# ai4r/Gesture-Generation-from-Trimodal-Context

Measured on AMD Instinct MI355X. Metric: training clips/sec (34-frame, 27-dim pose), post-warm-up GAN iteration, higher is better.
Workload: dtype f32; 1 GPU; multimodal_context GAN training iteration (BASELINE.json configs[1]), epoch > loss_warmup; batch_per_gpu=128, global_batch=128, frames=34, pose_dim=27, audio_samples=36267, n_words=20000, hipgraph=True, parallelism=dp1

## Files before the change

gesture-generation-from-trimodal-context_amd/_lib.py:

```python
import ctypes as C
import os

_HERE = os.path.dirname(os.path.abspath(__file__))
LIB_PATH = os.environ.get("TG_LIB_PATH") or os.path.join(_HERE, "libtrimodal_hip.so")


class Window(C.Structure):
    _fields_ = [("ptr", C.c_void_p), ("batch_stride", C.c_int64), ("row_stride", C.c_int64), ("rows_in", C.c_int32),
                ("rows_out", C.c_int32), ("row_step", C.c_int32), ("shift", C.c_int32), ("dil", C.c_int32),
                ("cw", C.c_int32), ("K", C.c_int32)]


P, I32, I64, F32, U32 = C.c_void_p, C.c_int32, C.c_int64, C.c_float, C.c_uint32
WP = C.POINTER(Window)


class NtProblem(C.Structure):
    _fields_ = [("A", Window), ("Bw", P), ("ldb", I64), ("b_seg_k", I32), ("reserved", I32), ("b_seg_stride", I64), ("bias", P), ("C", P),
                ("c_batch_stride", I64), ("c_row_stride", I64), ("c_rows_out", I32), ("M", I32), ("N", I32), ("act_slope", F32),
                ("accumulate", I32), ("out_scale", P), ("b_planes", P), ("b_plane_stride", I64), ("b_rows", I32), ("b_row0", I32),
                ("gate", P), ("res", P), ("C2", P), ("res_slope", F32), ("drop_site", U32), ("drop_state", P), ("drop_index0", I64),
                ("drop_p", F32), ("reserved4", I32), ("b_planes_kind", I32), ("reserved5", I32), ("b_inv_scale", P), ("a_row_scale", P), ("a_rowmax", P), ("c_rowmax", P), ("c2_rowmax", P), ("a_rowmax_rows", I32), ("reserved6", I32)]


# ... 24 lines not shown
    "tg_gemm_tn": [P, I64, WP, P, I64, I32, I32, I32, P, P, I64, P],
    "tg_colsum": [P, I64, I32, I32, P, I32, P],
    "tg_gru_forward": [P, I64, P, P, P, P, P, P, I64, I32, I32, I32, P],
    "tg_gru_backward": [P, P, P, I64, P, P, P, P, I64, P, I32, I32, I32, P],
    "tg_gru_h64_forward": [P, I64, P, P, P, P, P, P, I64, P, P, I32, I32, P],
    "tg_gru_h64_backward": [P, P, P, P, I64, P, P, P, P, I64, I32, I32, P],
    "tg_gru_forward_cluster": [P, I64, P, P, P, P, P, P, I64, P, P, P, I64, I32, I32, I32, P],
    "tg_gru_forward_cluster_rows": [P, I64, P, P, P, P, P, P, I64, P, P, P, I64, I32, I32, I32, I32, I32, P],
    "tg_gru_forward_vec": [P, I64, P, P, P, P, P, P, I64, I32, I32, I32, P],
    "tg_gru_backward_cluster": [P, P, P, P, I64, P, P, P, P, I64, P, I64, I32, I32, I32, P],
    "tg_gru_backward_cluster_stats": [P, P, P, P, I64, P, P, P, P, I64, P, I64, I32, I32, I32, P, I64, P, P, P],
    "tg_bn_train_stats": [P, I32, I32, I32, P, P, P, P, P, P, F32, F32, I32, P],
    "tg_bn_eval_stats": [P, P, I32, F32, P, P, P],
    "tg_bn_train_fused": [P, P, I32, I32, I32, P, P, P, P, P, P, P, F32, F32, F32, I32, P],
    "tg_bn_apply": [P, P, I32, I32, I32, P, P, P, P, F32, P],
    "tg_bn2_train": [P, P, I32, I32, I32, P, I64, P, P, P, P, P, P, P, F32, F32, F32, I32, P],
    "tg_bn2_backward": [P, P, P, I32, I32, I32, P, P, P, P, F32, P, I64, P, P, P],
    "tg_bn_backward": [P, P, P, I32, I32, P, P, P, P, F32, P, P, P, P],
    "tg_wav_front_stats": [P, I64, I32, I32, P, P, I32, I32, I32, P, I64, P, P, P, P, P, P, F32, F32, I32, P],
    "tg_wav_front_apply": [P, I64, I32, I32, P, P, I32, I32, I32, P, P, P, P, F32, P, P, P],
    "tg_wav_front_backward": [P, P, P, I64, I32, I32, P, P, I32, I32, I32, P, P, P, P, F32, P, I64, P, P, P, P, P],
    "tg_wav_front_backward_fused": [P, I32, P, P, P, I64, I32, I32, P, P, I32, I32, I32, P, P, P, P, F32, P, I64, P, P, P, P, P],
    "tg_speaker_fwd": [P, P, I32, P, P, P, P, P, P, P, P, P, P, P, P, I32, P, I64, I32, P, U32, P],
    "tg_speaker_bwd": [P, P, P, P, P, P, P, P, I32, P, P, P, P, P, P, P, P, P, P, I32, P],
    "tg_wav_conv2_wgrad": [P, P, I32, I32, I32, P, I64, P, P, P],
    "tg_out_mlp_compose": [P, P, P, P, I32, I32, I32, I32, P, P, P, P],
    "tg_out_mlp_param_grads": [P, P, P, P, P, I32, I32, I32, I32, P, P, P, P, P],
    "tg_zero": [P, I64, P],
    "tg_permute3_batch": [P, I32, I32, P],
    "tg_add_relu": [P, P, P, I64, P],
    "tg_act_mask_bwd": [P, P, P, F32, P, I64, P],
    "tg_act_mask_bwd2": [P, P, P, P, F32, P, P, I64, P],
    "tg_embed_gather_drop": [P, P, P, I32, I32, I32, F32, P, U32, P],
    "tg_d_preconv_bwd": [P] * 26 + [I32, P, I64, I32, I32, P],
    "tg_d_preconv_fwd": [P] * 27 + [I64, I32, I32, F32, F32, P],
    "tg_iter_head": [P, P, P, P, P, P, I64, I32, I32, I32, I32, I32, P, P, P, P, I32, P, U32, P, P, P],
    "tg_act_mask_bwd_drop": [P, P, F32, P, U32, I64, F32, P, I64, P],
    "tg_act_mask_bwd2_drop": [P, P, P, F32, P, U32, I64, F32, P, P, I64, P],
    "tg_mul": [P, P, P, I64, P],
    "tg_axpy": [P, P, F32, I32, I64, P],
    "tg_copy2d": [P, I64, P, I64, I32, I32, I32, P],
    "tg_repeat_rows": [P, I64, P, I64, I32, I32, I32, P],
    "tg_sum_rows": [P, I64, P, I64, I32, I32, I32, I32, P],
    "tg_add_halves": [P, P, I32, I32, P],
    "tg_sum_parts": [P, I64, I32, P, I64, P],
    "tg_narrow8_pair": [P, P, P, P, P, I32, I32, P],
    "tg_dup_halves": [P, P, I32, I32, P],
    "tg_make_pre_seq": [P, P, I32, I32, I32, I32, P],
    "tg_embed_gather": [P, P, P, I32, I32, I32, P],
    "tg_assemble_batch": [P, P, P, P, P, P, P, P, P, P, I32, I32, I32, I32, I32, I32, P, P, P, P, P],
    "tg_embed_scatter_add": [P, P, P, I32, I32, I32, P],
    "tg_permute3": [P, P, I32, I32, I32, I32, I32, I32, P],
    "tg_conv_dgrad_pack": [P, P, I32, I32, I32, I32, P],
    "tg_weight_norm_fwd": [P, P, P, I32, I32, I32, P],
    "tg_weight_norm_fwd_batch": [I32, C.POINTER(P), C.POINTER(P), C.POINTER(P), C.POINTER(P), I32, I32, I32, P],
    "tg_weight_norm_bwd": [P, P, P, P, P, I32, I32, I32, P],
    "tg_weight_norm_bwd_batch": [I32, C.POINTER(P), C.POINTER(P), C.POINTER(P), C.POINTER(P), C.POINTER(P), I32, I32, I32, P],
    "tg_rng_advance": [P, P],
    "tg_iter_begin": [P, P, P, P, P],
    "tg_dropout_mask": [P, I64, F32, P, U32, P],
    "tg_dropout_apply": [P, P, P, I64, F32, P, U32, P],
    "tg_normal": [P, I64, P, U32, P],
    "tg_randperm": [P, I32, P, U32, P],
    "tg_gather_i64": [P, P, P, I32, P],
    "tg_reparam_fwd": [P, P, P, P, I64, P],
    "tg_reparam_bwd": [P, P, P, P, P, I64, P],
# ... 138 lines not shown
```

gesture-generation-from-trimodal-context_amd/engine.py:

```python

import os
import zlib

import torch

from . import layers as L
from . import ops, _lib
from .ops import Win
from .params import ParamSlab

WAV_CONVS = ((0, 16, 1, 5, 1600), (3, 32, 16, 6, 0), (6, 64, 32, 6, 0), (9, 32, 64, 6, 0))
WAV_KW = 15


class DeviceRNG:

    def __init__(self, seed, device):
        self.state = ops.new_rng_state(seed, device)
        self._sites = {}

    def site(self, name):
        sid = self._sites.get(name)
        if sid is None:
            sid = (zlib.crc32(name.encode()) & 0x7FFFFFFF) or 1
# ... 81 lines not shown
        self.p_drop = module.dropout_prob
        self.pose_dim = module.pose_dim
        self.T = module.pre_length + module.gen_length
        ctx = module.input_context
        assert ctx in ("both", "audio", "text", "none"), ctx
        self.use_audio, self.use_text = ctx in ("both", "audio"), ctx in ("both", "text")
        self.z_mode = None if not module.z_obj else ("speaker" if module.speaker_embedding is not None else "random")
        D = self.pose_dim
        self.c_audio = D + 1
        self.c_text = self.c_audio + 32 * self.use_audio
        self.c_z = self.c_text + 32 * self.use_text
        self.in_size = self.c_z + (16 if self.z_mode else 0)

    def forward(self, pre_seq, in_text, in_audio, vid, *, training, groups=1, save=False, inject=None, tag="g", save_rows=None, out_into=None,
                side_work=None, side_head=None):
        P, G, Bf = self.views()
        Bs, T = in_text.shape
        H, D = self.H, self.pose_dim
        assert T == self.T and pre_seq.shape == (Bs, T, D + 1) and Bs % groups == 0
        tp = {"Bs": Bs, "groups": groups, "training": training}
        in_size = self.in_size
        pre_in_place = (pre_seq.stride() == (T * in_size, in_size, 1) and pre_seq.storage_offset() == 0 and
                        pre_seq.untyped_storage().nbytes() >= Bs * T * in_size * 4)
        in_data = pre_seq.as_strided((Bs, T, in_size), (T * in_size, in_size, 1)) if pre_in_place else L.empty(Bs, T, in_size, like=pre_seq)
        fork = L.Fork(pre_seq.device, enabled=(self.use_side_stream and self.use_audio) or self._audio_fork_on())
        self._side_work_ran = False
        self._w21_early = None
        L.prep_zone("pre_join")
        if self.use_audio:
            self._audio_fwd(P, Bf, in_audio, in_data, self.c_audio, tp, fork, training, groups, side_work, side_head)
        elif training and self.use_text:
            self._audio_fwd(P, Bf, in_audio, L.empty(Bs, T, 32, like=pre_seq), 0, {}, fork, training, groups, side_work, side_head)
        if self.use_text:
            self._text_fwd(P, in_text, in_data, tp, training, inject, tag)
        mu = logvar = z = None
        z_in_place = False
        if self.z_mode == "speaker":
            assert vid is not None
            draw = None
            if inject is not None and f"{tag}.eps" in inject:
                eps = inject[f"{tag}.eps"].contiguous()
            elif ops.SPEAKER_FUSED:
                eps, draw = L.empty(Bs, 16, like=pre_seq), (self.rng.state, self.rng.site(f"{tag}.eps"))
            else:
                eps = ops.normal(L.empty(Bs, 16, like=pre_seq), self.rng.state, self.rng.site(f"{tag}.eps"))
            if ops.SPEAKER_FUSED:
                se, zc, mu, logvar, z = ops.speaker_fwd(P["speaker_embedding.0.weight"], vid.contiguous(), P["speaker_embedding.1.weight"],
                                                        P["speaker_embedding.1.bias"], P["speaker_mu.weight"], P["speaker_mu.bias"],
                                                        P["speaker_logvar.weight"], P["speaker_logvar.bias"], eps,
                                                        rep=in_data.view(Bs * T, in_size)[:, self.c_z:], T=T, draw=draw)
                z_in_place = True
            else:
                se = ops.embed_gather(P["speaker_embedding.0.weight"], vid.contiguous(), L.empty(Bs, 16, like=pre_seq))
                zc = L.linear_fwd(se, P["speaker_embedding.1.weight"], P["speaker_embedding.1.bias"])
                mu = L.linear_fwd(zc, P["speaker_mu.weight"], P["speaker_mu.bias"])
                logvar = L.linear_fwd(zc, P["speaker_logvar.weight"], P["speaker_logvar.bias"])
                z = ops.reparam_fwd(mu, logvar, eps, torch.empty_like(mu))
            tp.update(se=se, zc=zc, mu=mu, logvar=logvar, eps=eps, vid=vid)
        elif self.z_mode == "random":
            if inject is not None and f"{tag}.z" in inject:
                z = inject[f"{tag}.z"].contiguous()
            else:
                z = ops.normal(L.empty(Bs, 16, like=pre_seq), self.rng.state, self.rng.site(f"{tag}.z"))

        fork.join()
        L.prep_zone("post_join")
        flat_in = in_data.view(Bs * T, in_size)
# ... 44 lines not shown
            wp = L.pack_conv_weight(P[f"{fe}.{idx}.weight"])
            last = idx == 9
            if last and shared:
                Lo = L.conv_out_len(x.shape[1], WAV_KW, stride, pad)
                assert Lo == T, f"audio length gives {Lo} frames, expected {T}"
                a_win = Win.conv(x, WAV_KW, stride=stride, pad=pad, rows_out=Lo)
                probs = []
                for g in range(groups):
                    o = in_data[g * Ba:(g + 1) * Ba, :, ca:ca + 32]
                    probs.append(dict(A=a_win, W=wp, bias=P[f"{fe}.{idx}.bias"], out=o, c_batch_stride=o.stride(0), c_row_stride=o.stride(1), c_rows_out=Lo))
                ops.gemm_nt_group(probs)
                wav.append((x, None, None))
                break
            out = in_data[:, :, ca:ca + 32] if last else None
            c = L.conv_fwd(x, wp, P[f"{fe}.{idx}.bias"], WAV_KW, stride=stride, pad=pad, out=out)
            if last:
                assert c.shape[1] == T, f"audio length gives {c.shape[1]} frames, expected {T}"
                wav.append((x, None, None))
                break
            y, st = L.bn_fwd(c, P[f"{fe}.{idx + 1}.weight"], P[f"{fe}.{idx + 1}.bias"], Bf[f"{fe}.{idx + 1}.running_mean"],
                             Bf[f"{fe}.{idx + 1}.running_var"], Bf[f"{fe}.{idx + 1}.num_batches_tracked"],
                             training=training, groups=1 if shared else groups, act_slope=0.3,
                             repeats=groups if shared else 1)
            wav.append((x, st, c.shape[1]))
            x = y
        if side_work is not None and fork.enabled:
            side_work()
            self._side_work_ran = True
        if fork.enabled and ops.OUT_MLP_COMPOSED and self.early_out_compose:
            self._w21_early = L.frozen(("w21", P["out.0.weight"].data_ptr()), lambda: ops.out_mlp_compose(P["out.0.weight"], P["out.0.bias"], P["out.2.weight"], P["out.2.bias"], dup=2))
        fork.__exit__(None, None, None)
        tp["wav"], tp["wav_shared"] = wav, shared

    def _text_fwd(self, P, in_text, in_data, tp, training, inject, tag):
        Bs, T, in_size = in_data.shape
        te = "text_encoder"
        E = P[f"{te}.embedding.weight"].shape[1]
        if (training and self.tcn_drop_regen and Bs * T >= 8192 and E % 4 == 0 and P[f"{te}.embedding.weight"].data_ptr() % 16 == 0 and
                not (inject is not None and f"{tag}.emb_drop" in inject)):
            cur, emb_mask = ops.embed_gather_drop(P[f"{te}.embedding.weight"], in_text.contiguous().view(-1), L.empty(Bs, T, E, like=in_data), 0.1,
                                                  self.rng.state, self.rng.site(f"{tag}.emb_drop"))
        else:
            emb = ops.embed_gather(P[f"{te}.embedding.weight"], in_text.contiguous().view(-1), L.empty(Bs, T, E, like=in_data))
            cur, emb_mask = self._drop(f"{tag}.emb_drop", emb, 0.1, inject) if training else (emb, None)
        names = [f"{te}.tcn.network.{i}.{c}" for i in range(self.n_layers) for c in ("conv1", "conv2")]
        wps, wts = L.frozen(("tcn_wn", P[names[0] + ".weight_v"].data_ptr(), training),
                            lambda: ops.weight_norm_fwd_batch([P[n + ".weight_v"] for n in names], [P[n + ".weight_g"] for n in names], want_t=training))
        Co_w = wps.shape[1]
        w_pl = ops.split_planes(wps.view(len(names) * Co_w, wps.shape[2])) if (ops.GEMM_PLANES and Bs * T >= 8192) else None
        sites = [f"{tag}.tcn{i}.drop{ci + 1}" for i in range(self.n_layers) for ci in range(2)]
        masks = [None] * len(sites)
        if training:
            if inject is not None and all(sn in inject for sn in sites):
                masks = [inject[sn].contiguous() for sn in sites]
            elif self.p_drop > 0.0 and self.tcn_drop_regen and Bs * T >= 8192 and wps.shape[1] % 4 == 0:
                per = Bs * T * wps.shape[1]
                site = self.rng.site(f"{tag}.tcn.drop")
                masks = [inject[sn].contiguous() if (inject is not None and sn in inject) else
                         ops.Drop(self.rng.state, site, self.p_drop, (Bs, T, wps.shape[1]), index0=j * per) for j, sn in enumerate(sites)]
            elif self.p_drop > 0.0:
                drawn = ops.dropout_mask(L.empty(len(sites), Bs, T, wps.shape[1], like=in_data), self.p_drop, self.rng.state,
                                         self.rng.site(f"{tag}.tcn.drop"))
                masks = [inject[sn].contiguous() if (inject is not None and sn in inject) else drawn[j] for j, sn in enumerate(sites)]
        tcn = []
        fuse_res = wps.shape[1] == cur.shape[2] and cur.is_contiguous() and ops.nt_ext_supported(
            Win.conv(cur, 2, pad=1, dil=1, rows_out=T), wps[0], cur, c_batch_stride=cur.stride(0), c_row_stride=cur.stride(1), c_rows_out=T)
        chain = (w_pl is not None and w_pl.kind == "h2" and fuse_res and cur.is_contiguous()
                 and ops.nt_kernel_plan([dict(A=Win.conv(cur, 2, pad=1, dil=1, rows_out=T), W=wps[0], bias=None, out=cur, c_batch_stride=cur.stride(0),
                                              c_row_stride=cur.stride(1), c_rows_out=T, w_planes=w_pl, a_rowmax=cur.view(-1))])[0] == 2)
        if chain:
            rmax = ops.zeros(1 + 2 * self.n_layers, Bs * T, device=cur.device)
            rm_in = ops.win_row_absmax(Win.conv(cur, 2, pad=1, dil=1, rows_out=T), out=rmax[0])
        for i in range(self.n_layers):
            d = 2 ** i
            blk = {"x": cur, "d": d}
            h = cur
            y = None
            for ci in range(2):
                j = 2 * i + ci
                m = masks[j]
                if m is not None:
                    assert m.shape == (Bs, T, wps.shape[1]), (sites[j], m.shape)
                sc = {}
                if chain:
                    rm_o1 = rmax[1 + self.n_layers + i]
                    sc = dict(a_rowmax=rm_in, out_rowmax=rm_o1) if ci == 0 else dict(a_rowmax=rm_o1, out2_rowmax=rmax[1 + i])
                if ci == 1 and fuse_res:
                    y = torch.empty_like(cur)
                    o = L.conv_fwd(h, wps[j], P[names[j] + ".bias"], 2, pad=d, dil=d, rows_out=T, act_slope=0.0, out_scale=m, res=cur, out2=y,
                                   res_slope=0.0, w_planes=w_pl, w_row0=j * Co_w, **sc)
                    if chain:
                        rm_in = rmax[1 + i]
                else:
                    o = L.conv_fwd(h, wps[j], P[names[j] + ".bias"], 2, pad=d, dil=d, rows_out=T, act_slope=0.0, out_scale=m, w_planes=w_pl,
                                   w_row0=j * Co_w, **sc)
                blk[f"in{ci}"], blk[f"wt{ci}"], blk[f"o{ci}"], blk[f"m{ci}"] = h, (wts[j] if wts is not None else None), o, m
# ... 403 lines not shown
```

gesture-generation-from-trimodal-context_amd/ops.py:

```python
import ctypes as C

import contextlib
import os

import torch

from . import _lib
from ._lib import Window, call


def _stream():
    return C.c_void_p(torch.cuda.current_stream().cuda_stream)


def _f32(t, name="tensor"):
    if not (isinstance(t, torch.Tensor) and t.is_cuda and t.dtype == torch.float32):
        raise TypeError(f"{name}: expected a CUDA float32 tensor, got {type(t).__name__} "
                        f"{getattr(t, 'dtype', None)} {getattr(t, 'device', None)}")
    return t


def _p(t):
    return C.c_void_p(t.data_ptr()) if t is not None else C.c_void_p(0)

# ... 1210 lines not shown

def embed_gather(table, idx, out):
    _flat(table, "table"); _i64(idx, "idx"); _flat(out, "out")
    n_rows, D = table.shape
    assert out.numel() == idx.numel() * D
    call("tg_embed_gather", _p(table), _p(idx), _p(out), idx.numel(), D, n_rows, _stream()); return out


def assemble_batch(rec, out_text, out_audio, out_vec, out_vid, *, remove_word_timing=False):
    B, n_poses = out_text.shape
    A = out_audio.shape[1]
    Dp = out_vec.shape[2]
    assert out_text.dtype == torch.int64 and out_vid.dtype == torch.int64 and out_text.is_contiguous() and out_audio.is_contiguous() and out_vec.is_contiguous()
    assert tuple(out_audio.shape) == (B, A) and tuple(out_vec.shape) == (B, n_poses, Dp) and out_vid.numel() == B
    _f32(out_audio, "out_audio"); _f32(out_vec, "out_vec"); _f32(rec["audio"], "audio"); _f32(rec["vec"], "vec")
    Wmax = rec["word_idx"].shape[1]
    assert rec["audio_off"].numel() == B + 1 and rec["vec_off"].numel() == B + 1 and tuple(rec["word_idx"].shape) == (B, Wmax) == tuple(rec["word_onset"].shape)
    assert rec["word_idx"].dtype == torch.int64 and rec["word_onset"].dtype == torch.float64 and rec["times"].dtype == torch.float64
    assert rec["n_words"].dtype == torch.int32 and rec["n_ext"].dtype == torch.int32 and rec["vid"].dtype == torch.int64
    assert rec["audio"].numel() >= 1 and rec["vec"].numel() >= B * n_poses * Dp
    call("tg_assemble_batch", _p(rec["audio"]), _p(rec["audio_off"]), _p(rec["vec"]), _p(rec["vec_off"]), _p(rec["word_idx"]), _p(rec["word_onset"]),
         _p(rec["n_words"]), _p(rec["times"]), _p(rec["n_ext"]), _p(rec["vid"]), B, Wmax, n_poses, Dp, A, int(bool(remove_word_timing)),
         _p(out_text), _p(out_audio), _p(out_vec), _p(out_vid), _stream())


def embed_gather_drop(table, idx, out, p, state, site):
    _flat(table, "table"); _i64(idx, "idx"); _flat(out, "out")
    n_rows, D = table.shape
    assert out.numel() == idx.numel() * D and D % 4 == 0
    call("tg_embed_gather_drop", _p(table), _p(idx), _p(out), idx.numel(), D, n_rows, float(p), _p(_i64(state, "rng_state")), int(site), _stream())
    return out, Drop(state, site, p, out.shape)


def embed_scatter_add(dout, idx, dtable):
    _flat(dout, "dout"); _i64(idx, "idx"); _flat(dtable, "dtable")
    n_rows, D = dtable.shape
    assert dout.numel() == idx.numel() * D
    call("tg_embed_scatter_add", _p(dout), _p(idx), _p(dtable), idx.numel(), D, n_rows, _stream()); return dtable


def permute3(x, out, perm):
    _flat(x, "in"); _flat(out, "out"); assert x.dim() == 3 and out.numel() == x.numel()
    call("tg_permute3", _p(x), _p(out), *x.shape, *perm, _stream()); return out


def permute3_batch(desc, n_jobs, total_workgroups):
    assert desc.dtype == torch.int64 and desc.is_cuda and desc.is_contiguous() and tuple(desc.shape) == (n_jobs, 10)
    call("tg_permute3_batch", C.c_void_p(desc.data_ptr()), int(n_jobs), int(total_workgroups), _stream())


def conv_dgrad_pack(w, out, stride):
    _flat(w, "w"); _flat(out, "out"); Co, Ci, kw = w.shape
    J = (kw + stride - 1) // stride
    assert out.numel() == stride * Ci * J * Co
    call("tg_conv_dgrad_pack", _p(w), _p(out), Co, Ci, kw, stride, _stream()); return out


def weight_norm_fwd(v, g, w_packed):
    _flat(v, "v"); _flat(g, "g"); _flat(w_packed, "w"); Co, Ci, kw = v.shape
    assert g.numel() == Co and w_packed.numel() == v.numel()
    call("tg_weight_norm_fwd", _p(v), _p(g), _p(w_packed), Co, Ci, kw, _stream()); return w_packed


def weight_norm_fwd_batch(vs, gs, want_t=True):
    n = len(vs)
    Co, Ci, kw = vs[0].shape
# ... 660 lines not shown
```

include/trimodal_hip.h:

```cpp
#ifndef TRIMODAL_HIP_H
#define TRIMODAL_HIP_H

#include <stdint.h>

#ifdef __cplusplus
extern "C" {
#endif

#define TG_ABI_VERSION 11

int tg_version(void);

int tg_set_deterministic(int32_t on);
int tg_get_deterministic(void);
int tg_set_tn_workgroup_cap(int32_t n);
int tg_get_tn_workgroup_cap(void);
const char* tg_last_error(void);

int tg_set_math_mode(int32_t mode);
int tg_get_math_mode(void);

typedef struct tg_window {
    const float* ptr;
    int64_t batch_stride;
// ... 198 lines not shown
int tg_wav_conv2_wgrad(const float* dc2, const float* act, int32_t B, int32_t T1, int32_t T2, float* ws, int64_t ws_floats, float* dW2,
                       float* db2, void* stream);

int tg_add_relu(const float* a, const float* b, float* y, int64_t n, void* stream);
int tg_act_mask_bwd2(const float* dy, const float* y, const float* o, const float* mask, float slope, float* dsum, float* dc, int64_t n, void* stream);
int tg_act_mask_bwd(const float* dy, const float* y, const float* mask, float slope, float* dx, int64_t n,
                    void* stream);
int tg_act_mask_bwd_drop(const float* dy, const float* y, float p, const uint64_t* rng_state, uint32_t site, int64_t index0, float slope,
                         float* dx, int64_t n, void* stream);
int tg_act_mask_bwd2_drop(const float* dy, const float* y, const float* o, float p, const uint64_t* rng_state, uint32_t site, int64_t index0,
                          float slope, float* dsum, float* dc, int64_t n, void* stream);
int tg_mul(const float* x, const float* mask, float* y, int64_t n, void* stream);
int tg_zero(void* p, int64_t bytes, void* stream);
int tg_axpy(const float* x, float* y, float alpha, int32_t accumulate, int64_t n, void* stream);
int tg_copy2d(const float* src, int64_t lds, float* dst, int64_t ldd, int32_t rows, int32_t cols,
              int32_t accumulate, void* stream);
int tg_repeat_rows(const float* src, int64_t lds, float* dst, int64_t ldd, int32_t B, int32_t T, int32_t cols,
                   void* stream);
int tg_sum_rows(const float* src, int64_t lds, float* dst, int64_t ldd, int32_t B, int32_t T, int32_t cols,
                int32_t accumulate, void* stream);
int tg_add_halves(const float* y, float* o, int32_t M, int32_t H, void* stream);
int tg_sum_parts(const float* parts, int64_t stride, int32_t n_parts, float* out, int64_t n, void* stream);
int tg_narrow8_pair(const float* a0, const float* a1, const float* w0, const float* w1, float* out, int32_t M, int32_t K, void* stream);
int tg_dup_halves(const float* d_o, float* dy, int32_t M, int32_t H, void* stream);
int tg_make_pre_seq(const float* target, float* pre, int32_t B, int32_t T, int32_t D, int32_t n_pre, void* stream);
int tg_assemble_batch(const float* audio_raw, const int64_t* audio_off, const float* vec_raw, const int64_t* vec_off, const int64_t* word_idx,
                      const double* word_onset, const int32_t* n_words, const double* times, const int32_t* n_ext, const int64_t* vid_in, int32_t B, int32_t Wmax,
                      int32_t n_poses, int32_t pose_floats, int32_t audio_len, int32_t remove_word_timing, int64_t* out_text, float* out_audio,
                      float* out_vec, int64_t* out_vid, void* stream);
int tg_embed_gather(const float* table, const int64_t* idx, float* out, int32_t n_idx, int32_t D, int32_t n_rows,
                    void* stream);
int tg_embed_gather_drop(const float* table, const int64_t* idx, float* out, int32_t n_idx, int32_t D, int32_t n_rows, float p,
                         const uint64_t* rng_state, uint32_t site, void* stream);
int tg_embed_scatter_add(const float* dout, const int64_t* idx, float* dtable, int32_t n_idx, int32_t D,
                         int32_t n_rows, void* stream);
int tg_permute3(const float* in, float* out, int32_t d0, int32_t d1, int32_t d2, int32_t p0, int32_t p1,
                int32_t p2, void* stream);

int tg_permute3_batch(const int64_t* desc, int32_t n_jobs, int32_t total_workgroups, void* stream);
int tg_conv_dgrad_pack(const float* w, float* out, int32_t Co, int32_t Ci, int32_t kw, int32_t s, void* stream);

int tg_weight_norm_fwd(const float* v, const float* g, float* w_packed, int32_t Co, int32_t Ci, int32_t kw,
                       void* stream);
int tg_weight_norm_fwd_batch(int32_t n, const float* const* v, const float* const* g, float* const* w_packed, float* const* w_t,
                             int32_t Co, int32_t Ci, int32_t kw, void* stream);
int tg_weight_norm_bwd(const float* dw_packed, const float* v, const float* g, float* dg, float* dv, int32_t Co,
                       int32_t Ci, int32_t kw, void* stream);
int tg_weight_norm_bwd_batch(int32_t n, const float* const* dw_packed, const float* const* v, const float* const* g, float* const* dg,
                             float* const* dv, int32_t Co, int32_t Ci, int32_t kw, void* stream);

int tg_rng_advance(uint64_t* rng_state, void* stream);
int tg_iter_begin(uint64_t* rng_a, uint64_t* rng_b, int32_t* adam_step_a, int32_t* adam_step_b, void* stream);
int tg_iter_head(uint64_t* rng_a, uint64_t* rng_b, int32_t* adam_step_a, int32_t* adam_step_b, const float* target, float* pre_stacked, int64_t pre_ld,
                 int32_t B, int32_t T, int32_t D, int32_t n_pre, int32_t copies, const int64_t* text, int64_t* text_stacked, const int64_t* vid,
                 int64_t* vid_stacked, int32_t permute_last, const int64_t* perm_in, uint32_t perm_site, int64_t* perm_out, float* target_copy,
                 void* stream);
int tg_dropout_mask(float* mask, int64_t n, float p, const uint64_t* rng_state, uint32_t site, void* stream);
int tg_dropout_apply(const float* x, float* y, float* mask, int64_t n, float p, const uint64_t* rng_state, uint32_t site,
                     void* stream);
int tg_normal(float* out, int64_t n, const uint64_t* rng_state, uint32_t site, void* stream);
int tg_randperm(int64_t* out, int32_t n, const uint64_t* rng_state, uint32_t site, void* stream);
int tg_gather_i64(const int64_t* src, const int64_t* perm, int64_t* out, int32_t n, void* stream);

int tg_reparam_fwd(const float* mu, const float* logvar, const float* eps, float* z, int64_t n, void* stream);
int tg_reparam_bwd(const float* dz, const float* logvar, const float* eps, float* dmu, float* dlogvar, int64_t n,
                   void* stream);
// ... 137 lines not shown
```

Before: 29610 clips/s.

## Fuse text TCN forward blocks and decoder into one persistent LDS-resident kernel

Adds a single HIP kernel that runs all four text-encoder TCN residual blocks (8 dilated conv layers with bias, ReLU, dropout and residual) plus the 32-wide decoder for two clips per workgroup. Activations stay in LDS as split fp16 hi/lo planes and feed MFMA instructions, replacing the per-layer GEMM launches and their global-memory round trips. It writes the tape tensors the backward pass needs. The cost is a large-LDS kernel with one workgroup per CU, only 64 workgroups for batch 128, and a fixed shape envelope that falls back to the old path otherwise.

```diff
diff --git a/gesture-generation-from-trimodal-context_amd/_lib.py b/gesture-generation-from-trimodal-context_amd/_lib.py
--- a/gesture-generation-from-trimodal-context_amd/_lib.py
+++ b/gesture-generation-from-trimodal-context_amd/_lib.py
@@ -80,6 +80,7 @@
     "tg_act_mask_bwd": [P, P, P, F32, P, I64, P],
     "tg_act_mask_bwd2": [P, P, P, P, F32, P, P, I64, P],
     "tg_embed_gather_drop": [P, P, P, I32, I32, I32, F32, P, U32, P],
+    "tg_tcn_fwd_fused": [P, P, I64, I32, P, C.POINTER(P), P, P, P, U32, F32, I32, I32, I32, I32, P, P, P, I32, I32, P, I64, P],
     "tg_d_preconv_bwd": [P] * 26 + [I32, P, I64, I32, I32, P],
     "tg_d_preconv_fwd": [P] * 27 + [I64, I32, I32, F32, F32, P],
     "tg_iter_head": [P, P, P, P, P, P, I64, I32, I32, I32, I32, I32, P, P, P, P, I32, P, U32, P, P, P],
diff --git a/gesture-generation-from-trimodal-context_amd/csrc/tcn_fused.hip b/gesture-generation-from-trimodal-context_amd/csrc/tcn_fused.hip
--- /dev/null
+++ b/gesture-generation-from-trimodal-context_amd/csrc/tcn_fused.hip
@@ -0,0 +1,313 @@
+#include "common.hpp"
+#include <stdlib.h>
+#include <type_traits>
+
+namespace tg {
+
+constexpr int TF_T = 34, TF_C = 300, TF_R = 2, TF_ROWS = TF_R * TF_T, TF_MT = 5, TF_NTILES = 19, TF_BLOCKS = 4, TF_E = 32;
+constexpr int TF_ROWB = TF_C * 2;
+constexpr int TF_PLANE = TF_ROWS * TF_ROWB;
+constexpr int TF_X_OFF = 0, TF_PL_OFF = TF_ROWS * TF_C * 4, TF_ZERO_OFF = TF_PL_OFF + 2 * TF_PLANE, TF_RMAX_OFF = TF_ZERO_OFF + 16;
+constexpr int TF_LDS = TF_RMAX_OFF + 2 * TF_ROWS * 4;
+constexpr int TF_Q_TAP = TF_C / 4;
+static_assert(TF_LDS <= 163840 && TF_PL_OFF % 16 == 0 && TF_PLANE % 8 == 0 && TF_ROWB % 8 == 0, "LDS layout");
+
+typedef unsigned tf_u32x2 __attribute__((ext_vector_type(2)));
+typedef unsigned tf_u32x4 __attribute__((ext_vector_type(4)));
+
+struct TcnArgs {
+    const float* x0;
+    const unsigned char* wpl;
+    long wplane_b;
+    unsigned wslab_b;
+    int wzero_row;
+    const float* winv;
+    const float* bias[2 * TF_BLOCKS];
+    const float* dec_w;
+    const float* dec_b;
+    const uint64_t* drop;
+    unsigned site;
+    float p;
+    int clips;
+    float *o0, *o1, *y;
+    int save0, save1;
+    float* out;
+    long out_ld;
+};
+
+struct TfW { tg_f16x8 hi, lo; };
+
+template <int NJ>
+__device__ __forceinline__ void tcn_fwd_fused_body(const TcnArgs& a, unsigned char* const smem) {
+    float* const xres = reinterpret_cast<float*>(smem + TF_X_OFF);
+    unsigned char* const pl = smem + TF_PL_OFF;
+    unsigned* const rmax = reinterpret_cast<unsigned*>(smem + TF_RMAX_OFF);
+    constexpr int ZREL = TF_ZERO_OFF - TF_PL_OFF;
+    const int t = threadIdx.x, lane = t & 63;
+    const int wave = __builtin_amdgcn_readfirstlane(t >> 6);
+    const int r16 = lane & 15, kq = lane >> 4;
+    const int clip0 = blockIdx.x * TF_R;
+    const int nclip = a.clips - clip0 < TF_R ? a.clips - clip0 : TF_R;
+
+    auto store_planes = [&](int row, int col, const f32x4 v, float s) __attribute__((always_inline)) {
+        unsigned h0, l0, h1, l1;
+        h2_split2(v[0] * s, v[1] * s, h0, l0);
+        h2_split2(v[2] * s, v[3] * s, h1, l1);
+        unsigned char* const q = pl + row * TF_ROWB + col * 2;
+        *reinterpret_cast<tf_u32x2*>(q) = tf_u32x2{h0, h1};
+        *reinterpret_cast<tf_u32x2*>(q + TF_PLANE) = tf_u32x2{l0, l1};
+    };
+    auto absmax4 = [](unsigned m, const f32x4 v) __attribute__((always_inline)) {
+#pragma unroll
+        for (int q = 0; q < 4; ++q) { const float f = v[q]; const unsigned b = __float_as_uint(f) & 0x7fffffffu; m = m > b ? m : b; }
+        return m;
+    };
+
+    {
+        const f32x4* __restrict__ src = reinterpret_cast<const f32x4*>(a.x0 + (long)clip0 * (TF_T * TF_C));
+        const int live = nclip * (TF_T * TF_C / 4);
+        for (int i = t; i < TF_ROWS * TF_C / 4; i += 512) reinterpret_cast<f32x4*>(xres)[i] = i < live ? src[i] : f32x4{0.f, 0.f, 0.f, 0.f};
+        if (t < 4) reinterpret_cast<unsigned*>(smem + TF_ZERO_OFF)[t] = 0u;
+        if (t < TF_ROWS) rmax[t] = 0u;
+    }
+    __syncthreads();
+    for (int row = wave; row < TF_ROWS; row += 8) {
+        const float* xr = xres + row * TF_C;
+        const bool two = lane + 64 < TF_C / 4;
+        const f32x4 v0 = *reinterpret_cast<const f32x4*>(xr + 4 * lane);
+        const f32x4 v1 = two ? *reinterpret_cast<const f32x4*>(xr + 4 * (lane + 64)) : f32x4{0.f, 0.f, 0.f, 0.f};
+        const unsigned mx = wave_max_u32(absmax4(absmax4(0u, v0), v1));
+        const float s = h2_scale_of_exp(h2_exp_of_bits(mx));
+        if (lane == 0) rmax[TF_ROWS + row] = mx;
+        store_planes(row, 4 * lane, v0, s);
+        if (two) store_planes(row, 4 * (lane + 64), v1, s);
+    }
+    __syncthreads();
+
+    int rowoff1[TF_MT];
+    int tl[TF_MT];
+    int goff[TF_MT];
+    bool rowok[TF_MT], saved[TF_MT], gok[TF_MT];
+#pragma unroll
+    for (int i = 0; i < TF_MT; ++i) {
+        const int m = 16 * i + r16;
+        rowok[i] = m < TF_ROWS;
+        const int mm = rowok[i] ? m : 0;
+        const int c = mm >= TF_T ? 1 : 0;
+        tl[i] = mm - c * TF_T;
+        rowoff1[i] = rowok[i] ? m * TF_ROWB : -1;
+        gok[i] = rowok[i] && c < nclip;
+        const int clip = gok[i] ? clip0 + c : 0;
+        saved[i] = gok[i] && clip >= a.save0 && clip < a.save1;
+        goff[i] = (clip * TF_T + tl[i]) * TF_C;
+    }
+    const long per = (long)a.clips * (TF_T * TF_C);
+    const bool drop_on = a.drop != nullptr && a.p > 0.f;
+
+    f32x4 acc[2][TF_MT][NJ];
+
+    for (int j = 0; j < 2 * TF_BLOCKS; ++j) {
+        const int d = 1 << (j >> 1);
+        const bool second = j & 1;
+        int rowoff0[TF_MT];
+#pragma unroll
+        for (int i = 0; i < TF_MT; ++i) rowoff0[i] = (rowok[i] && tl[i] >= d) ? rowoff1[i] - d * TF_ROWB : -1;
+        unsigned woff[NJ];
+#pragma unroll
+        for (int jn = 0; jn < NJ; ++jn) {
+            const int n = 16 * (wave + 8 * jn) + r16;
+            woff[jn] = (unsigned)(n < TF_C ? j * TF_C + n : a.wzero_row) * 64u + (unsigned)kq * 16u;
+        }
+        auto load_w = [&](int s, TfW (&w)[NJ]) __attribute__((always_inline)) {
+            const unsigned char* __restrict__ base = a.wpl + (size_t)s * a.wslab_b;
+#pragma unroll
+            for (int jn = 0; jn < NJ; ++jn) {
+                w[jn].hi = *reinterpret_cast<const tg_f16x8*>(base + woff[jn]);
+                w[jn].lo = *reinterpret_cast<const tg_f16x8*>(base + a.wplane_b + woff[jn]);
+            }
+        };
+        auto slab = [&](auto tap_c, int s, const TfW (&w)[NJ]) __attribute__((always_inline)) {
+            constexpr int TAP = decltype(tap_c)::value;
+            int cb[2];
+            bool ok[2];
+#pragma unroll
+            for (int h = 0; h < 2; ++h) {
+                const int q = 8 * s + 2 * kq + h;
+                ok[h] = TAP == 0 ? q < TF_Q_TAP : (q >= TF_Q_TAP && q < 2 * TF_Q_TAP);
+                cb[h] = (q - TAP * TF_Q_TAP) * 8;
+            }
+#pragma unroll
+            for (int i = 0; i < TF_MT; ++i) {
+                const int ro = TAP ? rowoff1[i] : rowoff0[i];
+                tf_u32x2 xh[2], xl[2];
+#pragma unroll
+                for (int h = 0; h < 2; ++h) {
+                    const bool v = ok[h] && ro >= 0;
+                    xh[h] = *reinterpret_cast<const tf_u32x2*>(pl + (v ? ro + cb[h] : ZREL));
+                    xl[h] = *reinterpret_cast<const tf_u32x2*>(pl + (v ? ro + cb[h] + TF_PLANE : ZREL));
+                }
+                const tg_f16x8 fh = __builtin_bit_cast(tg_f16x8, tf_u32x4{xh[0][0], xh[0][1], xh[1][0], xh[1][1]});
+                const tg_f16x8 fl = __builtin_bit_cast(tg_f16x8, tf_u32x4{xl[0][0], xl[0][1], xl[1][0], xl[1][1]});
+#pragma unroll
+                for (int jn = 0; jn < NJ; ++jn) acc[TAP][i][jn] = __builtin_amdgcn_mfma_f32_16x16x32_f16(w[jn].lo, fh, acc[TAP][i][jn], 0, 0, 0);
+#pragma unroll
+                for (int jn = 0; jn < NJ; ++jn) acc[TAP][i][jn] = __builtin_amdgcn_mfma_f32_16x16x32_f16(w[jn].hi, fl, acc[TAP][i][jn], 0, 0, 0);
+#pragma unroll
+                for (int jn = 0; jn < NJ; ++jn) acc[TAP][i][jn] = __builtin_amdgcn_mfma_f32_16x16x32_f16(w[jn].hi, fh, acc[TAP][i][jn], 0, 0, 0);
+            }
+        };
+#pragma unroll
+        for (int q = 0; q < 2; ++q)
+#pragma unroll
+            for (int i = 0; i < TF_MT; ++i)
+#pragma unroll
+                for (int jn = 0; jn < NJ; ++jn) acc[q][i][jn] = f32x4{0.f, 0.f, 0.f, 0.f};
+
+        using tap0 = std::integral_constant<int, 0>;
+        using tap1 = std::integral_constant<int, 1>;
+        TfW w0[NJ], w1[NJ];
+        load_w(0, w0);
+        for (int s = 0; s < 10; s += 2) {
+            load_w(s + 1, w1);
+            slab(tap0{}, s, w0);
+            load_w(s + 2 < 10 ? s + 2 : 9, w0);
+            slab(tap0{}, s + 1, w1);
+        }
+        for (int s = 9; s < 19; s += 2) {
+            load_w(s + 1, w1);
+            slab(tap1{}, s, w0);
+            load_w(s + 2 < 19 ? s + 2 : 18, w0);
+            slab(tap1{}, s + 1, w1);
+        }
+
+        const unsigned* const rm_in = rmax + ((j + 1) & 1) * TF_ROWS;
+        unsigned* const rm_out = rmax + (j & 1) * TF_ROWS;
+        const float* __restrict__ bias = a.bias[j];
+        const float* __restrict__ winv = a.winv + j * TF_C;
+        float* __restrict__ const tape0 = (second ? a.o1 : a.o0) + (long)(j >> 1) * per;
+        float* __restrict__ const tape_y = a.y + (long)(j >> 1) * per;
+#pragma unroll
+        for (int i = 0; i < TF_MT; ++i) {
+            const int m = rowok[i] ? 16 * i + r16 : 0;
+            const float inv1 = h2_inv_of_exp(h2_exp_of_bits(rm_in[m]));
+            const float inv0 = h2_inv_of_exp(h2_exp_of_bits(rm_in[tl[i] >= d ? m - d : m]));
+            unsigned mx = 0u;
+#pragma unroll
+            for (int jn = 0; jn < NJ; ++jn) {
+                const int n = 16 * (wave + 8 * jn) + 4 * kq;
+                const bool cok = n < TF_C;
+                const int nn = cok ? n : 0;
+                const f32x4 iw = *reinterpret_cast<const f32x4*>(winv + nn);
+                const f32x4 bv = *reinterpret_cast<const f32x4*>(bias + nn);
+                f32x4 v = (acc[0][i][jn] * inv0) * iw + (acc[1][i][jn] * inv1) * iw + bv;
+#pragma unroll
+                for (int q = 0; q < 4; ++q) v[q] = v[q] > 0.f ? v[q] : 0.f;
+                if (drop_on) v *= dropout_scale4(a.drop, a.site, a.p, (unsigned long)(j * per + goff[i] + nn) >> 2);
+                if (saved[i] && cok) *reinterpret_cast<f32x4*>(tape0 + goff[i] + nn) = v;
+                if (second) {
+                    float* const xp = xres + m * TF_C + nn;
+                    const f32x4 x = *reinterpret_cast<const f32x4*>(xp);
+                    v += x;
+#pragma unroll
+                    for (int q = 0; q < 4; ++q) v[q] = v[q] > 0.f ? v[q] : 0.f;
+                    if (rowok[i] && cok) *reinterpret_cast<f32x4*>(xp) = v;
+                    if (saved[i] && cok) *reinterpret_cast<f32x4*>(tape_y + goff[i] + nn) = v;
+                }
+                if (cok) mx = absmax4(mx, v);
+                acc[1][i][jn] = v;
+            }
+            unsigned o = (unsigned)__shfl_xor((int)mx, 16, 64); mx = mx > o ? mx : o;
+            o = (unsigned)__shfl_xor((int)mx, 32, 64); mx = mx > o ? mx : o;
+            if (kq == 0 && rowok[i]) atomicMax(rm_out + m, mx);
+        }
+        __syncthreads();
+        if (j == 2 * TF_BLOCKS - 1) break;
+        if (t < TF_ROWS) rmax[((j + 1) & 1) * TF_ROWS + t] = 0u;
+#pragma unroll
+        for (int i = 0; i < TF_MT; ++i) {
+            const int m = rowok[i] ? 16 * i + r16 : 0;
+            const float s = h2_scale_of_exp(h2_exp_of_bits(rm_out[m]));
+#pragma unroll
+            for (int jn = 0; jn < NJ; ++jn) {
+                const int n = 16 * (wave + 8 * jn) + 4 * kq;
+                if (rowok[i] && n < TF_C) store_planes(m, n, acc[1][i][jn], s);
+            }
+        }
+        __syncthreads();
+    }
+
+    {
+        const int c = t & 31, mg = t >> 5;
+        const float* __restrict__ wr = a.dec_w + c * TF_C;
+        float s[TF_MT];
+        int mrow[TF_MT];
+#pragma unroll
+        for (int k = 0; k < TF_MT; ++k) { s[k] = 0.f; const int m = mg + 16 * k; mrow[k] = (m < TF_ROWS ? m : 0) * TF_C; }
+        for (int k4 = 0; k4 < TF_C; k4 += 4) {
+            const f32x4 w = *reinterpret_cast<const f32x4*>(wr + k4);
+#pragma unroll
+            for (int k = 0; k < TF_MT; ++k) {
+                const f32x4 x = *reinterpret_cast<const f32x4*>(xres + mrow[k] + k4);
+                s[k] = fmaf(w[0], x[0], s[k]); s[k] = fmaf(w[1], x[1], s[k]); s[k] = fmaf(w[2], x[2], s[k]); s[k] = fmaf(w[3], x[3], s[k]);
+            }
+        }
+        const float b = a.dec_b[c];
+#pragma unroll
+        for (int k = 0; k < TF_MT; ++k) {
+            const int m = mg + 16 * k;
+            const int cl = m >= TF_T ? 1 : 0;
+            if (m < TF_ROWS && cl < nclip) a.out[((long)(clip0 + cl) * TF_T + (m - cl * TF_T)) * a.out_ld + c] = s[k] + b;
+        }
+    }
+}
+
+__global__ __launch_bounds__(512, 1) void tcn_fwd_fused_kernel(const TcnArgs a) {
+    __shared__ __attribute__((aligned(16))) unsigned char smem[TF_LDS];
+    if (__builtin_amdgcn_readfirstlane(threadIdx.x >> 6) + 16 < TF_NTILES) tcn_fwd_fused_body<3>(a, smem);
+    else tcn_fwd_fused_body<2>(a, smem);
+}
+
+}
+
+using namespace tg;
+
+extern "C" int tg_get_math_mode(void);
+
+static bool tcn_fused_envelope(int T, int C, int n_blocks) { return T == TF_T && C == TF_C && n_blocks == TF_BLOCKS && tg_get_math_mode() == 0; }
+
+extern "C" int tg_tcn_fwd_fused(const float* x0, const void* w_planes, int64_t w_plane_stride, int32_t w_rows, const float* w_inv, const float* const* biases,
+                                const float* dec_w, const float* dec_b, const uint64_t* rng_state, uint32_t site, float p, int32_t clips, int32_t T,
+                                int32_t C, int32_t n_blocks, float* o0, float* o1, float* y, int32_t save_row0, int32_t save_rows, float* out,
+                                int64_t out_ld, void* stream) {
+    TG_REQUIRE(x0 && w_planes && w_inv && biases && dec_w && dec_b && out, "tg_tcn_fwd_fused: null argument");
+    TG_REQUIRE(clips > 0 && clips <= (1 << 16), "tg_tcn_fwd_fused: clips must be in [1, 2^16]");
+    TG_REQUIRE(tcn_fused_envelope(T, C, n_blocks), "tg_tcn_fwd_fused: envelope is T = %d, C = %d, %d blocks, fp32-accurate mode", TF_T, TF_C, TF_BLOCKS);
+    constexpr int cwp = (2 * TF_C + 31) / 32 * 32;
+    TG_REQUIRE(w_rows == 2 * TF_BLOCKS * TF_C && w_plane_stride == (int64_t)(w_rows + 1) * cwp,
+               "tg_tcn_fwd_fused: the weight planes must hold %d rows of %d columns (fp16 x 2, slab-tiled)", 2 * TF_BLOCKS * TF_C, 2 * TF_C);
+    TG_REQUIRE(p >= 0.f && p < 1.f && (p == 0.f || rng_state), "tg_tcn_fwd_fused: 0 <= p < 1, and a Philox state when p > 0");
+    TG_REQUIRE(save_row0 >= 0 && save_rows >= 0 && (int64_t)save_row0 + save_rows <= clips, "tg_tcn_fwd_fused: taped clips outside the batch");
+    TG_REQUIRE(save_rows == 0 || (o0 && o1 && y), "tg_tcn_fwd_fused: taped clips need o0 / o1 / y");
+    TG_REQUIRE(out_ld >= TF_E, "tg_tcn_fwd_fused: out_ld below the decoder width");
+    TG_REQUIRE(aligned16(x0) && aligned16(w_planes) && aligned16(w_inv) && aligned16(dec_w) && aligned16(o0) && aligned16(o1) && aligned16(y),
+               "tg_tcn_fwd_fused: 16-byte aligned operands");
+    TcnArgs a;
+    for (int j = 0; j < 2 * TF_BLOCKS; ++j) {
+        TG_REQUIRE(biases[j] && aligned16(biases[j]), "tg_tcn_fwd_fused: bias %d null or misaligned", j);
+        a.bias[j] = biases[j];
+    }
+    a.x0 = x0;
+    a.wpl = static_cast<const unsigned char*>(w_planes);
+    a.wplane_b = (long)w_plane_stride * 2;
+    a.wslab_b = (unsigned)(w_rows + 1) * 64u;
+    a.wzero_row = w_rows;
+    a.winv = w_inv;
+    a.dec_w = dec_w; a.dec_b = dec_b;
+    a.drop = p > 0.f ? rng_state : nullptr;
+    a.site = site; a.p = p; a.clips = clips;
+    a.o0 = o0; a.o1 = o1; a.y = y;
+    a.save0 = save_row0; a.save1 = save_row0 + save_rows;
+    a.out = out; a.out_ld = out_ld;
+    hipLaunchKernelGGL(tcn_fwd_fused_kernel, dim3((clips + TF_R - 1) / TF_R), dim3(512), 0, static_cast<hipStream_t>(stream), a);
+    return check_launch("tg_tcn_fwd_fused");
+}
diff --git a/gesture-generation-from-trimodal-context_amd/engine.py b/gesture-generation-from-trimodal-context_amd/engine.py
--- a/gesture-generation-from-trimodal-context_amd/engine.py
+++ b/gesture-generation-from-trimodal-context_amd/engine.py
@@ -137,7 +137,7 @@
         elif training and self.use_text:
             self._audio_fwd(P, Bf, in_audio, L.empty(Bs, T, 32, like=pre_seq), 0, {}, fork, training, groups, side_work, side_head)
         if self.use_text:
-            self._text_fwd(P, in_text, in_data, tp, training, inject, tag)
+            self._text_fwd(P, in_text, in_data, tp, training, inject, tag, save, save_rows)
         mu = logvar = z = None
         z_in_place = False
         if self.z_mode == "speaker":
@@ -248,7 +248,7 @@
         fork.__exit__(None, None, None)
         tp["wav"], tp["wav_shared"] = wav, shared
 
-    def _text_fwd(self, P, in_text, in_data, tp, training, inject, tag):
+    def _text_fwd(self, P, in_text, in_data, tp, training, inject, tag, save=True, save_rows=None):
         Bs, T, in_size = in_data.shape
         te = "text_encoder"
         E = P[f"{te}.embedding.weight"].shape[1]
@@ -278,6 +278,23 @@
                 drawn = ops.dropout_mask(L.empty(len(sites), Bs, T, wps.shape[1], like=in_data), self.p_drop, self.rng.state,
                                          self.rng.site(f"{tag}.tcn.drop"))
                 masks = [inject[sn].contiguous() if (inject is not None and sn in inject) else drawn[j] for j, sn in enumerate(sites)]
+        biases = [P[n + ".bias"] for n in names]
+        if (training and wps.shape[1] == E and all(m is None or isinstance(m, ops.Drop) for m in masks)
+                and ops.tcn_fused_takes(cur, w_pl, 2, self.n_layers, P[f"{te}.decoder.weight"], biases)):
+            nb, Cc = self.n_layers, wps.shape[1]
+            tape = tuple(L.empty(nb, Bs, T, Cc, like=cur) for _ in range(3)) if save else None
+            drop = next((m for m in masks if m is not None), None)
+            ops.tcn_fwd_fused(cur, w_pl, biases, P[f"{te}.decoder.weight"], P[f"{te}.decoder.bias"], in_data[:, :, self.c_text:self.c_text + 32],
+                              p=drop.p if drop is not None else 0.0, state=drop.state if drop is not None else None,
+                              site=drop.site if drop is not None else 0, save_rows=((0, Bs) if save_rows is None else save_rows) if save else None, tape=tape)
+            tcn, x = [], cur
+            for i in range(nb if save else 0):
+                o0, o1, y = tape[0][i], tape[1][i], tape[2][i]
+                tcn.append({"x": x, "d": 2 ** i, "in0": x, "wt0": wts[2 * i] if wts is not None else None, "o0": o0, "m0": masks[2 * i],
+                            "in1": o0, "wt1": wts[2 * i + 1] if wts is not None else None, "o1": o1, "m1": masks[2 * i + 1], "y": y})
+                x = y
+            tp["tcn"], tp["emb_mask"], tp["text_x"] = tcn, emb_mask, (x if save else None)
+            return
         tcn = []
         fuse_res = wps.shape[1] == cur.shape[2] and cur.is_contiguous() and ops.nt_ext_supported(
             Win.conv(cur, 2, pad=1, dil=1, rows_out=T), wps[0], cur, c_batch_stride=cur.stride(0), c_row_stride=cur.stride(1), c_rows_out=T)
diff --git a/gesture-generation-from-trimodal-context_amd/ops.py b/gesture-generation-from-trimodal-context_amd/ops.py
--- a/gesture-generation-from-trimodal-context_amd/ops.py
+++ b/gesture-generation-from-trimodal-context_amd/ops.py
@@ -1266,6 +1266,50 @@
     return out, Drop(state, site, p, out.shape)
 
 
+TCN_FUSED = os.environ.get("TG_TCN_FUSED", "1") != "0"
+TCN_FUSED_ENVELOPE = "T = 34, C = E = 300, kernel size 2, 4 blocks, decoder width 32, fp16 x 2 weight planes, fp32-accurate math mode, 16-byte aligned operands"
+
+
+def tcn_fused_takes(x0, w_pl, ksize, n_blocks, dec_w, biases=()):
+    if not (TCN_FUSED and gemm_h2() and w_pl is not None and w_pl.kind == "h2"):
+        return False
+    if not (x0.dim() == 3 and x0.is_contiguous() and x0.dtype == torch.float32 and x0.data_ptr() % 16 == 0):
+        return False
+    _, T, E = x0.shape
+    return (T == 34 and E == 300 and ksize == 2 and n_blocks == 4 and w_pl.rows == 2 * n_blocks * E and w_pl.cw == ksize * E
+            and tuple(dec_w.shape) == (32, E) and dec_w.is_contiguous() and dec_w.data_ptr() % 16 == 0
+            and all(b.is_contiguous() and b.numel() == E and b.data_ptr() % 16 == 0 for b in biases))
+
+
+def tcn_fwd_fused(x0, w_pl, biases, dec_w, dec_b, out, *, p=0.0, state=None, site=0, save_rows=None, tape=None):
+    _flat(x0, "x0"); _f32(out, "out"); _flat(dec_w, "dec_w"); _flat(dec_b, "dec_b")
+    clips, T, Cc = x0.shape
+    nb = len(biases) // 2
+    for b in biases:
+        _flat(b, "bias")
+    if len(biases) != 2 * nb or not tcn_fused_takes(x0, w_pl, 2, nb, dec_w, biases):
+        raise ValueError(f"tcn_fwd_fused: outside the envelope ({TCN_FUSED_ENVELOPE})")
+    assert dec_b.numel() == 32 and w_pl.inv.numel() >= w_pl.rows and w_pl.t.is_contiguous()
+    assert tuple(out.shape) == (clips, T, 32) and out.stride(2) == 1 and out.stride(0) == T * out.stride(1) and out.stride(1) >= 32
+    if (clips * T - 1) * out.stride(1) + 32 > _room(out):
+        raise ValueError("tcn_fwd_fused: out exceeds its tensor")
+    r0, rn = (0, 0) if save_rows is None else (int(save_rows[0]), int(save_rows[1]))
+    assert 0 <= r0 and 0 <= rn and r0 + rn <= clips
+    if rn:
+        assert tape is not None and len(tape) == 3
+        for tt in tape:
+            _flat(tt, "tape"); assert tuple(tt.shape) == (nb, clips, T, Cc) and tt.data_ptr() % 16 == 0
+    p = float(p)
+    assert 0.0 <= p < 1.0
+    if p > 0.0:
+        _i64(state, "rng_state"); assert state.numel() >= 2
+    bp = (C.c_void_p * len(biases))(*[b.data_ptr() for b in biases])
+    tp = tape if rn else (None, None, None)
+    call("tg_tcn_fwd_fused", _p(x0), C.c_void_p(w_pl.t.data_ptr()), w_pl.plane_stride, w_pl.rows, _p(w_pl.inv), bp, _p(dec_w), _p(dec_b),
+         _p(state) if p > 0.0 else None, int(site), p, clips, T, Cc, nb, _p(tp[0]), _p(tp[1]), _p(tp[2]), r0, rn, _p(out), out.stride(1), _stream())
+    return out
+
+
 def embed_scatter_add(dout, idx, dtable):
     _flat(dout, "dout"); _i64(idx, "idx"); _flat(dtable, "dtable")
     n_rows, D = dtable.shape
diff --git a/include/trimodal_hip.h b/include/trimodal_hip.h
--- a/include/trimodal_hip.h
+++ b/include/trimodal_hip.h
@@ -254,6 +254,10 @@
                     void* stream);
 int tg_embed_gather_drop(const float* table, const int64_t* idx, float* out, int32_t n_idx, int32_t D, int32_t n_rows, float p,
                          const uint64_t* rng_state, uint32_t site, void* stream);
+int tg_tcn_fwd_fused(const float* x0, const void* w_planes, int64_t w_plane_stride, int32_t w_rows, const float* w_inv, const float* const* biases,
+                     const float* dec_w, const float* dec_b, const uint64_t* rng_state, uint32_t site, float p, int32_t clips, int32_t T, int32_t C,
+                     int32_t n_blocks, float* o0, float* o1, float* y, int32_t save_row0, int32_t save_rows, float* out, int64_t out_ld,
+                     void* stream);
 int tg_embed_scatter_add(const float* dout, const int64_t* idx, float* dtable, int32_t n_idx, int32_t D,
                          int32_t n_rows, void* stream);
 int tg_permute3(const float* in, float* out, int32_t d0, int32_t d1, int32_t d2, int32_t p0, int32_t p1,
```

Result: faster. 30160 clips/s (median of 6 runs) (+1.9%).
